# apachepinot/pinot

Measured on AMD Instinct MI355X. Metric: rows scanned/sec, 1B-row segment filter+groupby (3 predicates, SUM/MAX GROUP BY g1), higher is better.
Workload: dtype int64; 1 GPU; 1 segment(s) x 1000000000 rows, one per GPU; SELECT g1, SUM(m), MAX(m) FROM gpuBench WHERE c_inv1 IN (0,1,2,3) AND c_inv2 IN (0,1) AND r_int BETWEEN 250000 AND 749999 GROUP BY g1 ORDER BY g1 LIMIT 1000; query=cfg3, parallelism=segment-per-gpu x1, merge=none (1 segment), entries_scanned_in_filter=249990290

## Files before the change

pinot_amd/csrc/pg_kernels_spec.hip:

```cpp
#define PG_WAVES_PER_BLOCK 12
#define PG_KERNEL template <int PG_NOT_INSTANTIATED> static
#include "pg_kernels.hip"

#define SPEC_LOADERS 4
#ifndef SPEC_TILES
#define SPEC_TILES 2
#endif
#ifndef SPEC_SETS
#define SPEC_SETS 2
#endif
#define SPEC_CONSUMERS 8
#define SPEC_OFF_LIN 0u
#define SPEC_OFF_RNG 256u
#define SPEC_OFF_VAL (256u + 2048u)
#define SPEC_OFF_G0 (256u + 2048u + 8192u)
extern "C" const int pg_spec_waves_per_block = PG_WAVES_PER_BLOCK;
extern "C" int pg_spec_stage_bytes(int bits0, int bits1) { return SPEC_TILES * (((int)SPEC_OFF_G0 + bits0 * 256 + 16 + (bits1 > 0 ? bits1 * 256 + 16 : 0) + 15) & ~15); }

DEVFN void spec_barrier() {
  __builtin_amdgcn_fence(__ATOMIC_RELEASE, "workgroup", "local");
  __builtin_amdgcn_s_barrier();
  __builtin_amdgcn_fence(__ATOMIC_ACQUIRE, "workgroup", "local");
}

template <typename T> DEVFN const GAS T* spec_sgpr_ptr(const void* ptr) {
  const uint64_t v = (uint64_t)ptr;
  const uint32_t lo = (uint32_t)__builtin_amdgcn_readfirstlane((int)(uint32_t)v), hi = (uint32_t)__builtin_amdgcn_readfirstlane((int)(uint32_t)(v >> 32));
  return (const GAS T*)(((uint64_t)hi << 32) | (uint64_t)lo);
}

template <int W> struct SpecCol;
template <> struct SpecCol<0> {};
template <> struct SpecCol<32> { u32x4 r[2]; };
template <> struct SpecCol<24> { u32x4 lo; u32x2 hi; };
template <> struct SpecCol<16> { u32x4 lo; };
template <> struct SpecCol<8> { u32x2 hi; };
constexpr uint32_t spec_img_tile_bytes(int W) { return (uint32_t)(PG_WAVE_DOCS / 8) * (uint32_t)W; }
template <int W> DEVFN void spec_load(SpecCol<W>& c, const uint8_t* base, int wt, int w, int lane) {
  if constexpr (W == 32) {
#pragma unroll
    for (int s = 0; s < 2; s++) {
      const uint8_t* row = base + (size_t)wt * (PG_WAVE_DOCS * 4) + (size_t)(4 * s + w) * 1024u;
      c.r[s] = ldnt((const GAS u32x4*)(spec_sgpr_ptr<uint8_t>(row) + (uint32_t)lane * 16u));
    }
  } else if constexpr (W != 0) {
    const uint8_t* tile = base + (size_t)wt * spec_img_tile_bytes(W);
    if constexpr (W >= 16) c.lo = ldnt((const GAS u32x4*)(spec_sgpr_ptr<uint8_t>(tile + (size_t)w * 1024u) + (uint32_t)lane * 16u));
    if constexpr (W != 16) c.hi = ldnt((const GAS u32x2*)(spec_sgpr_ptr<uint8_t>(tile + (W == 24 ? 4096u : 0u) + (size_t)w * 512u) + (uint32_t)lane * 8u));
  }
}
template <int W> DEVFN void spec_unpack(const SpecCol<W>& c, uint32_t (&a)[4], uint32_t (&b)[4]) {
  if constexpr (W == 32) {
    a[0] = bswap32(c.r[0].x); a[1] = bswap32(c.r[0].y); a[2] = bswap32(c.r[0].z); a[3] = bswap32(c.r[0].w);
    b[0] = bswap32(c.r[1].x); b[1] = bswap32(c.r[1].y); b[2] = bswap32(c.r[1].z); b[3] = bswap32(c.r[1].w);
  } else if constexpr (W == 24) {
    a[0] = __builtin_amdgcn_perm(c.hi.x, c.lo.x, 0x0c040100u); a[1] = __builtin_amdgcn_perm(c.hi.x, c.lo.x, 0x0c050302u);
    a[2] = __builtin_amdgcn_perm(c.hi.x, c.lo.y, 0x0c060100u); a[3] = __builtin_amdgcn_perm(c.hi.x, c.lo.y, 0x0c070302u);
    b[0] = __builtin_amdgcn_perm(c.hi.y, c.lo.z, 0x0c040100u); b[1] = __builtin_amdgcn_perm(c.hi.y, c.lo.z, 0x0c050302u);
    b[2] = __builtin_amdgcn_perm(c.hi.y, c.lo.w, 0x0c060100u); b[3] = __builtin_amdgcn_perm(c.hi.y, c.lo.w, 0x0c070302u);
  } else if constexpr (W == 16) {
    a[0] = c.lo.x & 0xFFFFu; a[1] = c.lo.x >> 16; a[2] = c.lo.y & 0xFFFFu; a[3] = c.lo.y >> 16;
    b[0] = c.lo.z & 0xFFFFu; b[1] = c.lo.z >> 16; b[2] = c.lo.w & 0xFFFFu; b[3] = c.lo.w >> 16;
  } else if constexpr (W == 8) {
#pragma unroll
    for (int e = 0; e < 4; e++) { a[e] = (c.hi.x >> (8 * e)) & 0xFFu; b[e] = (c.hi.y >> (8 * e)) & 0xFFu; }
  }
}
template <int SW, int VW> struct SpecTile {
  SpecCol<SW> scan;
  SpecCol<VW> val;
  u32x4 grp;
};
template <int SW, int VW> struct SpecStage { SpecTile<SW, VW> tile[SPEC_TILES]; uint32_t post[8]; uint32_t tail; };
template <int NG> struct SpecQuad {
  uint32_t lin, rng;
  u32x4 val;
  uint32_t win[NG][2];
};

template <int W> struct SpecWidth { static constexpr int value = W; };
template <int NG, bool HAS_INDEX, bool HAS_SCAN, bool HAS_TAIL = false, bool NARROW = false>
__device__ __forceinline__ void spec_body(const PgQueryPlan& p) {
  extern __shared__ __attribute__((aligned(16))) uint64_t smem[];
  __shared__ uint32_t s_stat[PG_MAX_STATS];
  const int t = threadIdx.x;
  const int lane = t & 63;
  const int wave = uniform(t >> 6);
  int64_t* lds_table = reinterpret_cast<int64_t*>(smem);
  if (t < PG_MAX_STATS) s_stat[t] = 0;
  const uint32_t real_slots = (uint32_t)p.n_groups * (uint32_t)p.replicas;
  const uint32_t table_slots = real_slots + 64u;
  for (int o = 0; o < p.n_ops; o++) {
    const int64_t ident = pg_acc_identity(p.ops[o].fn, p.ops[o].is_float);
    for (uint32_t i = t; i < table_slots; i += PG_BLOCK) lds_table[(size_t)o * table_slots + i] = ident;
  }
  const uint32_t bits0 = (uint32_t)p.gcols[0].bits, bits1 = NG > 1 ? (uint32_t)p.gcols[NG - 1].bits : 0u;
  const uint32_t off_g1 = SPEC_OFF_G0 + bits0 * 256u + 16u;
  const uint32_t tile_bytes = (off_g1 + (NG > 1 ? bits1 * 256u + 16u : 0u) + 15u) & ~15u;
  const uint32_t stage_bytes = tile_bytes * SPEC_TILES;
  uint8_t* stage0 = reinterpret_cast<uint8_t*>(smem) + (((size_t)p.n_ops * table_slots * 8u + 15u) & ~(size_t)15u);
  const CAS PgScanLeaf& L = cptr(p.scans)[HAS_SCAN ? p.fast_scan : 0];
  const int grid = (int)gridDim.x;
  const int n_mine = (int)blockIdx.x < p.n_wtiles ? (p.n_wtiles - (int)blockIdx.x + grid - 1) / grid : 0;
  const int n_stages = (n_mine + SPEC_TILES - 1) / SPEC_TILES;
  __syncthreads();

  if (wave < SPEC_LOADERS) {
    const int w = wave;
    const uint8_t* const xdata = p.srcs[p.pipe_src].data;
    const uint8_t* const simg = NARROW ? p.spec_simg : nullptr;
    const uint8_t* const vimg = NARROW ? p.spec_vimg : nullptr;
    const uint32_t img_slo = NARROW ? p.spec_slo : 0u, img_sspan = NARROW ? p.spec_sspan : 0u, img_vmin = NARROW ? (uint32_t)p.spec_vmin : 0u;
    const bool img_sempty = NARROW && p.spec_sempty != 0;
    const int ggi = (w >> 1) < NG ? (w >> 1) : 0;
    const uint8_t* const gdata = p.gcols[ggi].data;
    const uint32_t gbits = (uint32_t)p.gcols[ggi].bits;
    const uint32_t goff = (uint32_t)(w & 1) * 1024u + (uint32_t)lane * 16u;
    const uint32_t geff = (w >> 1) < NG && goff < gbits * 256u ? goff : 0u;
    const uint8_t* dense_ptr[8];
    int dense_group[8];
#pragma unroll
    for (int j = 0; j < 8; j++) { dense_ptr[j] = HAS_INDEX ? p.dense_ptr[j] : nullptr; dense_group[j] = HAS_INDEX ? p.dense_group[j] : 0; }
    const int dense_groups = p.dense_groups, dense_excl = p.dense_excl;
    const uint8_t* const pipe_tail = HAS_TAIL ? p.pipe_tail : nullptr;
    const int num_docs = p.num_docs;
    const bool scan_pushed = p.fast_scan_pushed != 0;
   auto loaders = [&](auto scan_w, auto val_w) __attribute__((always_inline)) {
    constexpr int SW = HAS_SCAN ? decltype(scan_w)::value : 0, VW = decltype(val_w)::value;
    const RangeI32 r32 = !HAS_SCAN ? RangeI32{0, 0u, false} : (SW == 32 ? make_range_i32(L.lo, L.hi) : RangeI32{(int32_t)img_slo, img_sspan, img_sempty});
    const uint8_t* sdata = !HAS_SCAN ? nullptr : (SW == 32 ? L.data : simg);
    const uint8_t* vdata = VW == 32 ? xdata : vimg;
    const uint32_t vmin = VW == 32 ? 0u : img_vmin;
    uint32_t ld_cand = 0;
    auto issue = [&](int sidx, SpecStage<SW, VW>& st) __attribute__((always_inline)) {
#pragma unroll
      for (int tt = 0; tt < SPEC_TILES; tt++) {
        const int i = sidx * SPEC_TILES + tt;
        const int wt = (int)blockIdx.x + (i < n_mine ? i : n_mine - 1) * grid;
        SpecTile<SW, VW>& tl = st.tile[tt];
        __builtin_amdgcn_sched_barrier(0);
        spec_load<SW>(tl.scan, sdata, wt, w, lane);
        spec_load<VW>(tl.val, vdata, wt, w, lane);
        __builtin_amdgcn_sched_barrier(0);
        {
          const uint8_t* base = gdata + (size_t)wt * (size_t)(PG_WAVE_DOCS / 8) * (size_t)gbits;
          tl.grp = ldnt((const GAS u32x4*)(spec_sgpr_ptr<uint8_t>(base) + geff));
        }
        __builtin_amdgcn_sched_barrier(0);
      }
      if (HAS_INDEX) {
        const int i = sidx * SPEC_TILES + (w % SPEC_TILES);
        const int wt = (int)blockIdx.x + (i < n_mine ? i : n_mine - 1) * grid;
#pragma unroll
        for (int j = 0; j < 8; j++) st.post[j] = *(const GAS uint32_t*)(spec_sgpr_ptr<uint8_t>(dense_ptr[j] + (size_t)wt * 256u) + (uint32_t)lane * 4u);
        __builtin_amdgcn_sched_barrier(0);
      }
      if (HAS_TAIL) {
        const int i = sidx * SPEC_TILES + (w % SPEC_TILES);
        const int wt = (int)blockIdx.x + (i < n_mine ? i : n_mine - 1) * grid;
        st.tail = *(const GAS uint32_t*)(spec_sgpr_ptr<uint8_t>(pipe_tail + (size_t)wt * 256u) + (uint32_t)lane * 4u);
        __builtin_amdgcn_sched_barrier(0);
      }
    };
    auto publish = [&](uint8_t* stage, const SpecStage<SW, VW>& st) __attribute__((always_inline)) {
#ifdef PG_SPEC_NO_PUBLISH
      {
        uint32_t acc = 0;
#pragma unroll
        for (int tt = 0; tt < SPEC_TILES; tt++) {
          uint32_t a[4] = {0u, 0u, 0u, 0u}, b[4] = {0u, 0u, 0u, 0u};
          spec_unpack<SW>(st.tile[tt].scan, a, b); acc += a[0] ^ b[3];
          spec_unpack<VW>(st.tile[tt].val, a, b); acc += a[0] ^ b[3];
          acc += st.tile[tt].grp.x;
        }
        if (acc == 0x12345678u) *reinterpret_cast<uint32_t*>(stage) = acc;
        return;
      }
#endif
#pragma unroll
      for (int tt = 0; tt < SPEC_TILES; tt++) {
        uint8_t* buf = stage + (uint32_t)tt * tile_bytes;
        const SpecTile<SW, VW>& tl = st.tile[tt];
        if (HAS_SCAN) {
          uint32_t q[2][4];
          spec_unpack<SW>(tl.scan, q[0], q[1]);
#pragma unroll
          for (int s = 0; s < 2; s++) {
            uint32_t m = (uint32_t)in_range_i32(r32, (int32_t)q[s][0]) | ((uint32_t)in_range_i32(r32, (int32_t)q[s][1]) << 1) |
                         ((uint32_t)in_range_i32(r32, (int32_t)q[s][2]) << 2) | ((uint32_t)in_range_i32(r32, (int32_t)q[s][3]) << 3);
            m = r32.empty ? 0u : m;
            *reinterpret_cast<uint32_t*>(buf + SPEC_OFF_RNG + (uint32_t)(4 * s + w) * 256u + (uint32_t)lane * 4u) = m;
          }
        }
        {
          uint32_t q[2][4];
          spec_unpack<VW>(tl.val, q[0], q[1]);
#pragma unroll
          for (int s = 0; s < 2; s++) {
            u32x4 v;
            v.x = q[s][0] + vmin; v.y = q[s][1] + vmin; v.z = q[s][2] + vmin; v.w = q[s][3] + vmin;
            *reinterpret_cast<u32x4*>(buf + SPEC_OFF_VAL + (uint32_t)(4 * s + w) * 1024u + (uint32_t)lane * 16u) = v;
          }
        }
        *reinterpret_cast<u32x4*>(buf + (ggi == 0 ? SPEC_OFF_G0 : off_g1) + geff) = tl.grp;
      }
    };
    auto publish_lin = [&](uint8_t* stage, const SpecStage<SW, VW>& st, int sidx) __attribute__((always_inline)) {
      if (w >= SPEC_TILES) return;
      const int i = sidx * SPEC_TILES + w;
      const int wt = (int)blockIdx.x + i * grid;
      const int64_t rem = i < n_mine ? (int64_t)num_docs - (int64_t)wt * PG_WAVE_DOCS : 0;
      const int32_t n_valid = rem >= PG_WAVE_DOCS ? PG_WAVE_DOCS : (rem > 0 ? (int32_t)rem : 0);
      uint32_t lin = valid_lin_mask(n_valid, lane);
      if (HAS_INDEX) {
        uint32_t grp[4] = {0u, 0u, 0u, 0u};
#pragma unroll
        for (int j = 0; j < 8; j++) {
          const int gj = dense_group[j];
#pragma unroll
          for (int k = 0; k < 4; k++) grp[k] |= gj == k ? st.post[j] : 0u;
        }
#pragma unroll
        for (int k = 0; k < 4; k++)
          if (k < dense_groups) lin &= ((dense_excl >> k) & 1) ? ~grp[k] : grp[k];
      }
      *reinterpret_cast<uint32_t*>(stage + (uint32_t)w * tile_bytes + SPEC_OFF_LIN + (uint32_t)lane * 4u) = HAS_TAIL ? lin & st.tail : lin;
      ld_cand += (uint32_t)__popc(lin);
    };
    constexpr int SETS = HAS_SCAN ? SPEC_SETS : 2 * SPEC_SETS;
    SpecStage<SW, VW> st[SETS];
    auto buf_of = [&](int sg) __attribute__((always_inline)) { return stage0 + (uint32_t)(sg & 1) * stage_bytes; };
    if (n_stages > 0) {
#pragma unroll
      for (int k = 0; k < SETS; k++) issue(k, st[k]);
    }
    int s = 0;
    for (; s + SETS - 1 < n_stages; s += SETS) {
#pragma unroll
      for (int k = 0; k < SETS; k++) {
        publish(buf_of(s + k), st[k]);
        publish_lin(buf_of(s + k), st[k], s + k);
        issue(s + k + SETS, st[k]);
        spec_barrier();
      }
    }
#pragma unroll
    for (int k = 0; k < SETS - 1; k++)
      if (s + k < n_stages) {
        publish(buf_of(s + k), st[k]);
        publish_lin(buf_of(s + k), st[k], s + k);
        spec_barrier();
      }
    const uint32_t csum = wave_sum_u32(ld_cand);
    if (HAS_SCAN && !scan_pushed && lane == 0 && csum) atomicAdd(&s_stat[L.stat_slot], csum);
   };
    if constexpr (!NARROW) {
      loaders(SpecWidth<32>{}, SpecWidth<32>{});
    } else {
      const int sb = uniform(p.spec_sbits), vb = uniform(p.spec_vbits);
      auto with_scan = [&](auto scan_w) __attribute__((always_inline)) {
        switch (vb) {
          case 8: loaders(scan_w, SpecWidth<8>{}); break;
          case 16: loaders(scan_w, SpecWidth<16>{}); break;
          case 24: loaders(scan_w, SpecWidth<24>{}); break;
          default: loaders(scan_w, SpecWidth<32>{}); break;
        }
      };
      switch (sb) {
        case 8: with_scan(SpecWidth<8>{}); break;
        case 16: with_scan(SpecWidth<16>{}); break;
        case 24: with_scan(SpecWidth<24>{}); break;
        default: with_scan(SpecWidth<32>{}); break;
      }
    }
  } else {
    const int c = wave - SPEC_LOADERS;
    const uint32_t R = (uint32_t)p.replicas;
    const uint32_t rep = (uint32_t)t & (R - 1u);
    const uint32_t stride = table_slots;
    const uint32_t trash_slot = real_slots + (uint32_t)lane;
    const uint32_t q = (uint32_t)c * 64u + (uint32_t)lane;
    const uint32_t nib = ((uint32_t)lane & 7u) * 4u;
    uint32_t my_matched = 0;
    const int n_ops = uniform(p.n_ops);
    uint64_t ops_code = 0;
    for (int o = 0; o < n_ops; o++) {
      const PgAccOp op = p.ops[uniform(o)];
      ops_code |= (uint64_t)(op.src < 0 ? 0u : (op.fn == PG_ACC_SUM ? 1u : (op.fn == PG_ACC_MIN ? 2u : 3u))) << (2 * o);
    }
    ops_code = ((uint64_t)(uint32_t)uniform((int)(uint32_t)(ops_code >> 32)) << 32) | (uint64_t)(uint32_t)uniform((int)(uint32_t)ops_code);
    const int has_out_words = uniform(p.out_words != nullptr ? 1 : 0);
    auto fetch = [&](const uint8_t* buf, SpecQuad<NG>& d) __attribute__((always_inline)) {
      d.lin = *reinterpret_cast<const uint32_t*>(buf + SPEC_OFF_LIN + (q >> 3) * 4u);
      d.rng = HAS_SCAN ? *reinterpret_cast<const uint32_t*>(buf + SPEC_OFF_RNG + q * 4u) : 0xFu;
      d.val = *reinterpret_cast<const u32x4*>(buf + SPEC_OFF_VAL + q * 16u);
#pragma unroll
      for (int gi = 0; gi < NG; gi++) {
        const uint32_t di = __umul24(4u * q, (uint32_t)p.gcols[gi].bits) >> 5;
        const uint32_t* win = reinterpret_cast<const uint32_t*>(buf + (gi == 0 ? SPEC_OFF_G0 : off_g1)) + di;
        d.win[gi][0] = win[0]; d.win[gi][1] = win[1];
      }
    };
    auto aggregate = [&](const SpecQuad<NG> (&d)[SPEC_TILES], int sidx) __attribute__((always_inline)) {
      constexpr int ND = 4 * SPEC_TILES;
      uint32_t slot[ND];
      int32_t v[ND];
#pragma unroll
      for (int tt = 0; tt < SPEC_TILES; tt++) {
        const int i = sidx * SPEC_TILES + tt;
        const uint32_t cand = (d[tt].lin >> nib) & 0xFu;
        const uint32_t m = d[tt].rng & cand;
        my_matched += (uint32_t)__popc(m);
        if (has_out_words && i < n_mine) {
          const int wt = (int)blockIdx.x + i * grid;
          const uint32_t word = or_reduce8(m << nib);
          if ((lane & 7) == 0) reinterpret_cast<uint32_t*>(p.out_words)[(int64_t)wt * 64 + (int64_t)(q >> 3)] = word;
        }
#ifndef PG_SPEC_NO_TABLE
#pragma unroll
        for (int e = 0; e < 4; e++) slot[4 * tt + e] = rep;
#pragma unroll
        for (int gi = 0; gi < NG; gi++) {
          const PgGroupCol& gc = p.gcols[gi];
          const uint32_t bits = (uint32_t)gc.bits, mask = (1u << gc.bits) - 1u;
          const uint32_t mult = (uint32_t)gc.mult * R;
          uint32_t dv[4];
          decode_packed_quad<true>(d[tt].win[gi], q, bits, mask, dv);
#pragma unroll
          for (int e = 0; e < 4; e++) slot[4 * tt + e] += __umul24(dv[e], mult);
        }
#pragma unroll
        for (int e = 0; e < 4; e++) slot[4 * tt + e] = ((m >> e) & 1u) ? slot[4 * tt + e] : trash_slot;
        v[4 * tt + 0] = (int32_t)d[tt].val.x; v[4 * tt + 1] = (int32_t)d[tt].val.y; v[4 * tt + 2] = (int32_t)d[tt].val.z; v[4 * tt + 3] = (int32_t)d[tt].val.w;
#endif
      }
#ifdef PG_SPEC_NO_TABLE
      return;
#endif
      for (int o = 0; o < n_ops; o++) {
        const uint32_t code = (uint32_t)(ops_code >> (2 * o)) & 3u;
        int64_t* base = lds_table + (size_t)o * stride;
        if (code == 0u) {
#pragma unroll
          for (int e = 0; e < ND; e++) atomicAdd(reinterpret_cast<unsigned long long*>(base + slot[e]), 1ULL);
        } else if (code == 1u) {
#pragma unroll
          for (int e = 0; e < ND; e++) atomicAdd(reinterpret_cast<unsigned long long*>(base + slot[e]), (unsigned long long)(int64_t)v[e]);
        } else if (code == 2u) {
#pragma unroll
          for (int e = 0; e < ND; e++) atomicMin(reinterpret_cast<long long*>(base + slot[e]), (long long)v[e]);
        } else {
#pragma unroll
          for (int e = 0; e < ND; e++) atomicMax(reinterpret_cast<long long*>(base + slot[e]), (long long)v[e]);
        }
      }
    };
    auto fetch_stage = [&](int sidx, SpecQuad<NG> (&d)[SPEC_TILES]) __attribute__((always_inline)) {
      const uint8_t* stage = stage0 + (uint32_t)(sidx & 1) * stage_bytes;
#pragma unroll
      for (int tt = 0; tt < SPEC_TILES; tt++) fetch(stage + (uint32_t)tt * tile_bytes, d[tt]);
    };
    auto aggregate_stage = [&](int sidx, const SpecQuad<NG> (&d)[SPEC_TILES]) __attribute__((always_inline)) {
#ifdef PG_SPEC_NO_CONSUME
      return;
#endif
#ifdef PG_SPEC_FETCH_ONLY
      {
        uint32_t acc = 0;
#pragma unroll
        for (int tt = 0; tt < SPEC_TILES; tt++) { acc += d[tt].lin ^ d[tt].rng ^ d[tt].val.x ^ d[tt].val.w; for (int gi = 0; gi < NG; gi++) acc += d[tt].win[gi][0] ^ d[tt].win[gi][1]; }
        if (acc == 0x12345678u) my_matched++;
        return;
      }
#endif
      aggregate(d, sidx);
    };
    SpecQuad<NG> da[SPEC_TILES], db[SPEC_TILES];
    if (n_stages > 0) {
      spec_barrier();
#ifndef PG_SPEC_NO_CONSUME
      fetch_stage(0, da);
#endif
    }
    for (int s = 0; s < n_stages; s += 2) {
      if (s + 1 < n_stages) {
        spec_barrier();
#ifndef PG_SPEC_NO_CONSUME
        fetch_stage(s + 1, db);
#endif
      }
      aggregate_stage(s, da);
      if (s + 1 < n_stages) {
        if (s + 2 < n_stages) {
          spec_barrier();
#ifndef PG_SPEC_NO_CONSUME
          fetch_stage(s + 2, da);
#endif
        }
        aggregate_stage(s + 1, db);
      }
    }
    const uint32_t wsum = wave_sum_u32(my_matched);
    if (lane == 0 && wsum) atomicAdd(&s_stat[0], wsum);
  }
  __syncthreads();
  if (t < PG_MAX_STATS && s_stat[t]) atomicAdd(&p.stats[t], (unsigned long long)s_stat[t]);
  {
    const int R = p.replicas, groups = p.n_groups;
    int64_t* out = p.partials + (int64_t)blockIdx.x * ((int64_t)p.n_ops * groups);
    for (int o = 0; o < p.n_ops; o++) {
      const int fn = p.ops[uniform(o)].fn;
      for (int gq = t; gq < groups; gq += PG_BLOCK) {
        const int64_t* src = lds_table + (size_t)o * table_slots + (size_t)gq * R;
        int64_t acc = src[0];
        if (fn == PG_ACC_COUNT || fn == PG_ACC_SUM) { for (int r = 1; r < R; r++) acc += src[r]; }
        else if (fn == PG_ACC_MIN) { for (int r = 1; r < R; r++) acc = src[r] < acc ? src[r] : acc; }
        else { for (int r = 1; r < R; r++) acc = src[r] > acc ? src[r] : acc; }
        out[(size_t)o * groups + gq] = acc;
      }
    }
  }
}
#define PG_SPEC_KERNEL(NAME, IDX, SCAN) \
  extern "C" __global__ void __launch_bounds__(PG_BLOCK) NAME(const PgQueryPlan p) { \
    if (p.n_group_cols == 1) spec_body<1, IDX, SCAN>(p); \
    else spec_body<2, IDX, SCAN>(p); \
  }
PG_SPEC_KERNEL(pg_spec_none, false, false)
PG_SPEC_KERNEL(pg_spec_scan, false, true)
PG_SPEC_KERNEL(pg_spec_index, true, false)
#undef PG_SPEC_KERNEL
extern "C" __global__ void __launch_bounds__(PG_BLOCK) pg_fast_i32range_s(const PgQueryPlan p) {
  if (p.n_group_cols == 1) spec_body<1, true, true, false, true>(p);
  else spec_body<2, true, true, false, true>(p);
}
extern "C" __global__ void __launch_bounds__(PG_BLOCK) pg_fast_i32range_st(const PgQueryPlan p) {
  if (p.n_group_cols == 1) spec_body<1, true, true, true, true>(p);
  else spec_body<2, true, true, true, true>(p);
}
```

pinot_amd/csrc/pg_segment.cpp:

```cpp
#include <hip/hip_runtime.h>

#include <algorithm>
#include <cmath>

#include "pg_internal.hpp"

extern "C" __global__ void __launch_bounds__(256) pg_column_magnitude_kernel(const uint8_t* __restrict__ data, int64_t n, int val_type,
                                                                             unsigned long long* __restrict__ out) {
  unsigned long long mx = 0, bad = 0;
  for (int64_t i = (int64_t)blockIdx.x * blockDim.x + threadIdx.x; i < n; i += (int64_t)gridDim.x * blockDim.x) {
    unsigned long long a;
    if (val_type == PG_V_I64) {
      const unsigned long long v = __builtin_bswap64(reinterpret_cast<const unsigned long long*>(data)[i]);
      a = (long long)v < 0 ? 0ULL - v : v;
    } else {
      double d;
      if (val_type == PG_V_F32) d = (double)__uint_as_float(__builtin_bswap32(reinterpret_cast<const uint32_t*>(data)[i]));
      else d = __longlong_as_double((long long)__builtin_bswap64(reinterpret_cast<const unsigned long long*>(data)[i]));
      a = (unsigned long long)__double_as_longlong(d) & 0x7FFFFFFFFFFFFFFFULL;
      if (a >= 0x7FF0000000000000ULL) { bad = 1; a = 0; }
    }
    mx = a > mx ? a : mx;
  }
  for (int off = 32; off > 0; off >>= 1) {
    const unsigned long long o = __shfl_xor(mx, off, 64);
    mx = o > mx ? o : mx;
    bad |= __shfl_xor(bad, off, 64);
  }
  if ((threadIdx.x & 63) == 0) {
    if (mx) atomicMax(&out[0], mx);
    if (bad) atomicOr(&out[1], 1ULL);
  }
}

extern "C" __global__ void __launch_bounds__(256) pg_column_int_range_kernel(const uint8_t* __restrict__ data, int64_t n, int val_type,
                                                                             long long* __restrict__ out) {
  long long mn = INT64_MAX, mx = INT64_MIN;
  for (int64_t i = (int64_t)blockIdx.x * blockDim.x + threadIdx.x; i < n; i += (int64_t)gridDim.x * blockDim.x) {
    const long long v = val_type == PG_V_I64 ? (long long)__builtin_bswap64(reinterpret_cast<const unsigned long long*>(data)[i])
                                             : (long long)(int32_t)__builtin_bswap32(reinterpret_cast<const uint32_t*>(data)[i]);
    mn = v < mn ? v : mn;
    mx = v > mx ? v : mx;
  }
  for (int off = 32; off > 0; off >>= 1) {
    const long long a = __shfl_xor(mn, off, 64), b = __shfl_xor(mx, off, 64);
    mn = a < mn ? a : mn;
    mx = b > mx ? b : mx;
  }
  if ((threadIdx.x & 63) == 0 && mn <= mx) {
    atomicMin(&out[0], mn);
    atomicMax(&out[1], mx);
  }
}

extern "C" __global__ void __launch_bounds__(256) pg_column_narrow_image_kernel(const uint8_t* __restrict__ data, uint8_t* __restrict__ img,
                                                                                int64_t n_wtiles, int32_t vmin, int bits) {
  const int64_t n = n_wtiles * 256;
  const int64_t tile_bytes = (int64_t)(PG_WAVE_DOCS / 8) * bits;
  for (int64_t i = (int64_t)blockIdx.x * blockDim.x + threadIdx.x; i < n; i += (int64_t)gridDim.x * blockDim.x) {
    const int64_t wt = i >> 8;
    const int b = (int)(i >> 6) & 3, l = (int)i & 63;
    const uint4 qa = *reinterpret_cast<const uint4*>(data + wt * (PG_WAVE_DOCS * 4) + (int64_t)b * 1024 + l * 16);
    const uint4 qb = *reinterpret_cast<const uint4*>(data + wt * (PG_WAVE_DOCS * 4) + (int64_t)(4 + b) * 1024 + l * 16);
    const uint32_t raw[8] = {qa.x, qa.y, qa.z, qa.w, qb.x, qb.y, qb.z, qb.w};
    uint32_t s[8];
    for (int e = 0; e < 8; e++) s[e] = (__builtin_bswap32(raw[e]) - (uint32_t)vmin) & (bits == 24 ? 0xFFFFFFu : (bits == 16 ? 0xFFFFu : 0xFFu));
    uint8_t* tile = img + wt * tile_bytes;
    if (bits >= 16) {
      uint4 lo;
      lo.x = (s[0] & 0xFFFFu) | (s[1] << 16); lo.y = (s[2] & 0xFFFFu) | (s[3] << 16);
      lo.z = (s[4] & 0xFFFFu) | (s[5] << 16); lo.w = (s[6] & 0xFFFFu) | (s[7] << 16);
      *reinterpret_cast<uint4*>(tile + (int64_t)b * 1024 + l * 16) = lo;
    }
    if (bits != 16) {
      const int sh = bits == 24 ? 16 : 0;
      uint2 hi;
      hi.x = ((s[0] >> sh) & 0xFFu) | (((s[1] >> sh) & 0xFFu) << 8) | (((s[2] >> sh) & 0xFFu) << 16) | (((s[3] >> sh) & 0xFFu) << 24);
      hi.y = ((s[4] >> sh) & 0xFFu) | (((s[5] >> sh) & 0xFFu) << 8) | (((s[6] >> sh) & 0xFFu) << 16) | (((s[7] >> sh) & 0xFFu) << 24);
      *reinterpret_cast<uint2*>(tile + (bits == 24 ? 4096 : 0) + (int64_t)b * 512 + l * 8) = hi;
    }
  }
}

extern "C" __global__ void __launch_bounds__(256) pg_column_max_dict_id_kernel(const uint8_t* __restrict__ data, int64_t n, int bits,
                                                                                unsigned int* __restrict__ out) {
  unsigned int mx = 0;
  const uint64_t mask = (1ULL << bits) - 1ULL;
  for (int64_t i = (int64_t)blockIdx.x * blockDim.x + threadIdx.x; i < n; i += (int64_t)gridDim.x * blockDim.x) {
    const uint64_t bit = (uint64_t)i * (uint64_t)bits;
    const uint8_t* p = data + (bit >> 3);
    uint64_t w = 0;
    for (int k = 0; k < 8; k++) w = (w << 8) | p[k];
    const unsigned int v = (unsigned int)((w >> (64 - bits - (int)(bit & 7))) & mask);
    mx = v > mx ? v : mx;
  }
  for (int off = 32; off > 0; off >>= 1) {
    const unsigned int o = __shfl_xor(mx, off, 64);
    mx = o > mx ? o : mx;
  }
  if ((threadIdx.x & 63) == 0 && mx) atomicMax(out, mx);
}

namespace pg {

static int32_t fx_exp_of(double max_abs) {
  if (!(max_abs > 0)) return 0;
  int e = 0;
  (void)std::frexp(max_abs, &e);
  return (int32_t)(16 * (int)std::floor(((double)e + 15.0) / 16.0));
}

static inline uint32_t be32(const uint8_t* p) {
  return ((uint32_t)p[0] << 24) | ((uint32_t)p[1] << 16) | ((uint32_t)p[2] << 8) | (uint32_t)p[3];
}
static inline uint64_t be64(const uint8_t* p) { return ((uint64_t)be32(p) << 32) | be32(p + 4); }
static inline uint16_t le16(const uint8_t* p) { return (uint16_t)(p[0] | (p[1] << 8)); }
static inline uint32_t le32(const uint8_t* p) {
  return (uint32_t)p[0] | ((uint32_t)p[1] << 8) | ((uint32_t)p[2] << 16) | ((uint32_t)p[3] << 24);
}

Column* Segment::find(const char* n) {
  if (!n) return nullptr;
  auto it = columns.find(n);
  return it == columns.end() ? nullptr : it->second.get();
}

static size_t padded_docs(const Segment& seg) { return (size_t)seg.n_tiles * PG_TILE_DOCS; }

static void check_dict_ids(const Column& c, int64_t n) {
  if (n <= 0 || c.cardinality <= 0 || !(c.bits >= 31 || ((int64_t)1 << c.bits) > (int64_t)c.cardinality)) return;
  DeviceBuffer out(4, true);
  const int grid = (int)std::max<int64_t>(1, std::min<int64_t>(2048, (n + 255) / 256));
  hipLaunchKernelGGL(pg_column_max_dict_id_kernel, dim3(grid), dim3(256), 0, 0, c.fwd_dev.as<uint8_t>(), n, c.bits, out.as<unsigned int>());
  PG_HIP(hipGetLastError());
  unsigned int mx = 0;
  PG_HIP(hipMemcpy(&mx, out.ptr, 4, hipMemcpyDeviceToHost));
  if ((int64_t)mx >= (int64_t)c.cardinality)
    fail(PG_ERR_INVALID_ARGUMENT, "forward index of %s holds dictId %u, the dictionary has %d values", c.name.c_str(), mx, c.cardinality);
}

static void upload_fixed_bit(Segment& seg, Column& c, const uint8_t* src, uint64_t len) {
  uint64_t need = ((uint64_t)seg.total_docs * (uint64_t)c.bits + 7) / 8;
  if (len < need) fail(PG_ERR_INVALID_ARGUMENT, "forward index of %s is %llu bytes, need %llu", c.name.c_str(),
                       (unsigned long long)len, (unsigned long long)need);
  size_t alloc = (padded_docs(seg) * (size_t)c.bits + 7) / 8 + 64;
  c.fwd_dev.alloc(alloc, true);
  c.fwd_dev.upload(src, need);
  c.col_kind = PG_COL_FIXED_BIT;
  c.fwd_bytes_logical = need;
  check_dict_ids(c, (int64_t)seg.total_docs);
}

static void parse_inverted_index(Segment& seg, Column& c, const uint8_t* inv, uint64_t len) {
  const int32_t card = c.cardinality;
  const uint64_t off_end = ((uint64_t)card + 1) * 4;
  if (len < off_end) fail(PG_ERR_INVALID_ARGUMENT, "inverted index of %s too short", c.name.c_str());
  const uint64_t first = be32(inv);
  const uint8_t* bitmap_buffer = inv + off_end;
  c.posting_begin.assign((size_t)card + 1, 0);
  std::vector<uint8_t> staging;
  staging.reserve(len);
  const uint32_t max_key = (uint32_t)((padded_docs(seg) + PG_CHUNK_DOCS - 1) / PG_CHUNK_DOCS);
  c.posting_card.assign((size_t)card, 0);
  for (int32_t d = 0; d < card; d++) {
    c.posting_begin[d] = (uint32_t)c.descs_host.size();
    uint64_t off = be32(inv + (uint64_t)d * 4), end = be32(inv + (uint64_t)(d + 1) * 4);
    if (end < off || off < first || (end - first) > len - off_end)
      fail(PG_ERR_INVALID_ARGUMENT, "inverted index of %s: bad offsets for dictId %d", c.name.c_str(), d);
    const uint8_t* blob = bitmap_buffer + (off - first);
    uint64_t blen = end - off;
    if (blen < 8) fail(PG_ERR_INVALID_ARGUMENT, "roaring blob too short (%s dictId %d)", c.name.c_str(), d);
    uint32_t cookie = le32(blob);
    uint64_t pos = 4;
    uint32_t size;
    const uint8_t* run_flags = nullptr;
    bool has_run = false;
    if ((cookie & 0xFFFF) == 12347) {
      size = (cookie >> 16) + 1;
      run_flags = blob + pos;
      pos += (size + 7) / 8;
      has_run = true;
    } else if (cookie == 12346) {
      size = le32(blob + pos);
      pos += 4;
    } else {
      fail(PG_ERR_INVALID_ARGUMENT, "roaring: bad cookie %u (%s dictId %d)", cookie, c.name.c_str(), d);
    }
    if (pos + 4ULL * size > blen) fail(PG_ERR_INVALID_ARGUMENT, "roaring: truncated header");
    const uint8_t* desc = blob + pos;
    pos += 4ULL * size;
    if (!has_run || size >= 4) pos += 4ULL * size;
    for (uint32_t i = 0; i < size; i++) {
      PgContainer pc{};
      pc.key = le16(desc + 4 * i);
      uint32_t cardm1 = le16(desc + 4 * i + 2);
      bool is_run = has_run && ((run_flags[i >> 3] >> (i & 7)) & 1);
      uint64_t payload;
      if (is_run) {
        if (pos + 2 > blen) fail(PG_ERR_INVALID_ARGUMENT, "roaring: truncated run container");
        pc.n = le16(blob + pos);
        pos += 2;
        pc.type = 2;
        payload = 4ULL * pc.n;
      } else if (cardm1 + 1 > 4096) {
        pc.type = 1;
        pc.n = cardm1 + 1;
        payload = 8192;
      } else {
        pc.type = 0;
        pc.n = cardm1 + 1;
        payload = 2ULL * pc.n;
      }
      if (pos + payload > blen) fail(PG_ERR_INVALID_ARGUMENT, "roaring: truncated container");
      if (pc.type == 2) for (uint32_t r = 0; r < pc.n; r++) c.posting_card[(size_t)d] += (int64_t)le16(blob + pos + 4 * r + 2) + 1;
      else c.posting_card[(size_t)d] += pc.n;
      if (pc.key >= max_key) fail(PG_ERR_INVALID_ARGUMENT, "roaring: container key %u beyond the segment", pc.key);
      size_t aligned = (staging.size() + 15) & ~(size_t)15;
      staging.resize(aligned + payload);
      memcpy(staging.data() + aligned, blob + pos, payload);
      pc.offset = aligned;
      pos += payload;
      c.descs_host.push_back(pc);
    }
  }
  c.posting_begin[card] = (uint32_t)c.descs_host.size();
  staging.resize(((staging.size() + 15) & ~(size_t)15) + 16);
  c.containers_dev.alloc(staging.size());
  c.containers_dev.upload(staging.data(), staging.size());
  c.descs_dev = upload_vector(c.descs_host);
  c.has_inverted = true;
}

static std::shared_ptr<Column> bitmap_column(Segment& seg, const std::string& name, const void* roaring, uint64_t size) {
  if (!roaring || size < 8) fail(PG_ERR_INVALID_ARGUMENT, "%s: not a serialized RoaringBitmap", name.c_str());
  if (size > 0xFFFFFFF0ULL) fail(PG_ERR_UNSUPPORTED, "%s: bitmap larger than 4 GB", name.c_str());
  auto col = std::make_shared<Column>();
  col->name = name;
  col->cardinality = 1;
  std::vector<uint8_t> inv(8 + size);
  const uint32_t offs[2] = {8, (uint32_t)(8 + size)};
  for (int i = 0; i < 2; i++) for (int b = 0; b < 4; b++) inv[(size_t)i * 4 + b] = (uint8_t)(offs[i] >> (24 - 8 * b));
  memcpy(inv.data() + 8, roaring, size);
  parse_inverted_index(seg, *col, inv.data(), inv.size());
  return col;
}

void segment_set_null_vector(Segment& seg, const char* column, const void* roaring, uint64_t size) {
  if (!column || !seg.find(column)) fail(PG_ERR_NOT_FOUND, "column not found: %s", column ? column : "(null)");
  auto col = bitmap_column(seg, std::string("nullvalue_vector of ") + column, roaring, size);
  std::lock_guard<std::mutex> g(seg.mu);
  seg.null_vectors[column] = std::move(col);
  seg.plan_cache.clear();
}

void segment_set_range_index(Segment& seg, const char* column, const void* bytes, uint64_t size) {
  Column* c = column ? seg.find(column) : nullptr;
  if (!c) fail(PG_ERR_NOT_FOUND, "column not found: %s", column ? column : "(null)");
  const uint8_t* p = static_cast<const uint8_t*>(bytes);
  if (!p || size < 22) fail(PG_ERR_INVALID_ARGUMENT, "range index of %s too short", column);
  const int32_t version = (int32_t)be32(p);
  if (version != 2) fail(PG_ERR_UNSUPPORTED, "range index of %s: version %d (only the exact bit-sliced index, version 2, is on the GPU path)", column, version);
  const int64_t min = (int64_t)be64(p + 4);
  const uint8_t* r = p + 12;
  if (le16(r) != 0xF00D || r[2] != 2) fail(PG_ERR_INVALID_ARGUMENT, "range index of %s: bad RangeBitmap cookie / base", column);
  const int slices = r[3];
  const uint32_t max_key = le16(r + 4), max_rid = le32(r + 6);
  const int bytes_per_mask = (slices + 7) >> 3;
  if (slices < 1 || slices > 64) fail(PG_ERR_INVALID_ARGUMENT, "range index of %s: %d slices", column, slices);
  if ((int64_t)max_rid < (int64_t)seg.total_docs) fail(PG_ERR_INVALID_ARGUMENT, "range index of %s covers %u rows, the segment has %d", column, max_rid, seg.total_docs);
  const uint32_t n_chunks = (uint32_t)((padded_docs(seg) + PG_CHUNK_DOCS - 1) / PG_CHUNK_DOCS);
  if (max_key > n_chunks) fail(PG_ERR_INVALID_ARGUMENT, "range index of %s: %u chunks beyond the segment", column, max_key);
  uint64_t pos = 22 + (uint64_t)max_key * (uint64_t)bytes_per_mask;
  if (pos > size) fail(PG_ERR_INVALID_ARGUMENT, "range index of %s: truncated masks", column);
  std::vector<PgContainer> descs((size_t)n_chunks * (size_t)slices);
  for (auto& d : descs) { d.offset = 0; d.n = 0; d.key = 0; d.type = 3; }
  std::vector<uint8_t> staging;
  staging.reserve(size);
  for (uint32_t key = 0; key < max_key; key++) {
    uint64_t mask = 0;
    for (int b = 0; b < bytes_per_mask; b++) mask |= (uint64_t)p[22 + (uint64_t)key * bytes_per_mask + b] << (8 * b);
    for (int s = 0; s < slices; s++) {
      if (!((mask >> s) & 1)) continue;
      if (pos + 1 > size) fail(PG_ERR_INVALID_ARGUMENT, "range index of %s: truncated container", column);
      const int type = p[pos++];
      PgContainer pc{};
      pc.key = (uint16_t)key;
      uint64_t payload;
      if (type == 0) { pc.type = 1; pc.n = 0; payload = 8192; }
      else if (type == 1 || type == 2) {
        if (pos + 2 > size) fail(PG_ERR_INVALID_ARGUMENT, "range index of %s: truncated container", column);
        pc.n = le16(p + pos);
        pos += 2;
        pc.type = type == 1 ? 2 : 0;
        payload = type == 1 ? 4ULL * pc.n : 2ULL * pc.n;
      } else {
        fail(PG_ERR_INVALID_ARGUMENT, "range index of %s: container type %d", column, type);
      }
      if (pos + payload > size) fail(PG_ERR_INVALID_ARGUMENT, "range index of %s: truncated container", column);
      const size_t aligned = (staging.size() + 15) & ~(size_t)15;
      staging.resize(aligned + payload);
      memcpy(staging.data() + aligned, p + pos, payload);
      pc.offset = aligned;
      pos += payload;
      descs[(size_t)key * (size_t)slices + (size_t)s] = pc;
    }
  }
  staging.resize(((staging.size() + 15) & ~(size_t)15) + 16);
  DeviceBuffer cont(staging.size());
  cont.upload(staging.data(), staging.size());
  DeviceBuffer dd = upload_vector(descs);
  std::lock_guard<std::mutex> g(seg.mu);
  seg.device_bytes += cont.size + dd.size;
  c->ri_containers_dev = std::move(cont);
  c->ri_descs_dev = std::move(dd);
  c->ri_slices = slices;
  c->ri_chunks = (int32_t)n_chunks;
  c->ri_min = min;
  c->ri_bytes = size;
  c->has_range_index = true;
  seg.plan_cache.clear();
}

void segment_set_queryable_doc_ids(Segment& seg, const void* roaring, uint64_t size) {
  std::shared_ptr<Column> col;
  if (size) col = bitmap_column(seg, "queryableDocIds", roaring, size);
  std::lock_guard<std::mutex> g(seg.mu);
  seg.queryable_doc_ids = std::move(col);
  seg.plan_cache.clear();
}

template <typename F>
static void walk_var_byte_chunks(const Segment& seg, const uint8_t* fwd, uint64_t fwd_len, const char* name, bool pass_through_only, F each) {
  if (fwd_len < 28) fail(PG_ERR_INVALID_ARGUMENT, "raw forward index of %s too short", name);
  const int32_t version = (int32_t)be32(fwd), num_chunks = (int32_t)be32(fwd + 4), per_chunk = (int32_t)be32(fwd + 8);
  if (version != 2 && version != 3) fail(PG_ERR_UNSUPPORTED, "column %s: var-byte chunk writer version %d", name, version);
  const int32_t longest = (int32_t)be32(fwd + 12), compression = (int32_t)be32(fwd + 20), header_start = (int32_t)be32(fwd + 24);
  if (compression != 0 && pass_through_only)
    fail(PG_ERR_UNSUPPORTED, "column %s: compressed var-byte chunks (type %d) are outside the GPU path", name, compression);
  const int off_size = version == 2 ? 4 : 8;
  if (per_chunk <= 0 || num_chunks < 0 || longest < 0 || (int64_t)num_chunks * per_chunk < seg.total_docs || header_start < 28 ||
      (uint64_t)header_start + (uint64_t)num_chunks * (uint64_t)off_size > fwd_len)
    fail(PG_ERR_INVALID_ARGUMENT, "raw forward index of %s: %d chunks of %d docs for %d docs", name, num_chunks, per_chunk, seg.total_docs);
  const uint64_t max_chunk = (uint64_t)per_chunk * (4ULL + (uint64_t)longest);
  for (int32_t ch = 0; ch < num_chunks && (int64_t)ch * per_chunk < seg.total_docs; ch++) {
    auto chunk_pos = [&](int32_t i) -> uint64_t {
      if (i == num_chunks) return fwd_len;
      const uint8_t* o = fwd + header_start + (uint64_t)i * (uint64_t)off_size;
      return off_size == 4 ? (uint64_t)be32(o) : be64(o);
    };
    const uint64_t start = chunk_pos(ch), end = chunk_pos(ch + 1);
    if (start > end || end > fwd_len) fail(PG_ERR_INVALID_ARGUMENT, "raw forward index of %s: bad chunk offsets", name);
    std::vector<uint8_t> plain;
    const uint8_t* cb = fwd + start;
    uint64_t clen = end - start;
    if (compression != 0) {
      plain = host_decompress_chunk(compression, cb, clen, max_chunk, name);
      cb = plain.data();
      clen = plain.size();
    }
    if (clen < (uint64_t)per_chunk * 4) fail(PG_ERR_INVALID_ARGUMENT, "raw forward index of %s: chunk %d is %llu bytes", name, ch, (unsigned long long)clen);
    const int32_t rows = (int32_t)std::min<int64_t>(per_chunk, (int64_t)seg.total_docs - (int64_t)ch * per_chunk);
    for (int32_t r = 0; r < rows; r++) {
      const uint64_t vs = be32(cb + (size_t)r * 4);
      uint64_t ve = clen;
      if (r + 1 < per_chunk) { const uint64_t nx = be32(cb + (size_t)(r + 1) * 4); if (nx != 0) ve = nx; }
      if (vs < (uint64_t)per_chunk * 4 || ve < vs || ve > clen) fail(PG_ERR_INVALID_ARGUMENT, "raw forward index of %s: bad value offsets in chunk %d", name, ch);
      each((int64_t)ch * per_chunk + r, cb + vs, ve - vs);
    }
  }
}

void segment_add_column(Segment& seg, const pg_column_desc& d) {
  if (!d.name) fail(PG_ERR_INVALID_ARGUMENT, "column name is null");
  if (seg.columns.count(d.name)) fail(PG_ERR_INVALID_ARGUMENT, "column %s already added", d.name);
  auto col = std::make_unique<Column>();
  Column& c = *col;
  c.name = d.name;
  c.data_type = d.data_type;
  c.fwd_encoding = d.fwd_encoding;
  c.has_dictionary = d.has_dictionary != 0;
  c.cardinality = d.cardinality;
  c.bits = d.bits_per_value;
// ... 569 lines not shown
```

Baseline: 841.6 billion rows/s.

## Split narrow-image loaders by column and widen hi-byte loads to 16B

For narrow (8/16/24-bit) column images, the four loader waves are now split by column: two waves load the scan column and two load the value column, each covering one whole tile of a stage. Previously each loader loaded a slice of both columns. The image builder interleaves the high-byte plane so each lane can fetch it with 16-byte loads instead of 8-byte ones. The goal is fewer, wider global loads per wave and less unpack work per column. The cost is uneven work between the two roles, since only one role does the index/tail loads, and more registers held per stage.

Result: faster. 870.4 billion rows/s (median of 6 runs) (+3.4%).

```diff
diff --git a/pinot_amd/csrc/pg_kernels_spec.hip b/pinot_amd/csrc/pg_kernels_spec.hip
--- a/pinot_amd/csrc/pg_kernels_spec.hip
+++ b/pinot_amd/csrc/pg_kernels_spec.hip
@@ -8,6 +8,9 @@
 #endif
 #ifndef SPEC_SETS
 #define SPEC_SETS 2
+#endif
+#ifndef SPEC_INDEX_ROLE
+#define SPEC_INDEX_ROLE 0
 #endif
 #define SPEC_CONSUMERS 8
 #define SPEC_OFF_LIN 0u
@@ -32,9 +35,6 @@
 template <int W> struct SpecCol;
 template <> struct SpecCol<0> {};
 template <> struct SpecCol<32> { u32x4 r[2]; };
-template <> struct SpecCol<24> { u32x4 lo; u32x2 hi; };
-template <> struct SpecCol<16> { u32x4 lo; };
-template <> struct SpecCol<8> { u32x2 hi; };
 constexpr uint32_t spec_img_tile_bytes(int W) { return (uint32_t)(PG_WAVE_DOCS / 8) * (uint32_t)W; }
 template <int W> DEVFN void spec_load(SpecCol<W>& c, const uint8_t* base, int wt, int w, int lane) {
   if constexpr (W == 32) {
@@ -43,29 +43,53 @@
       const uint8_t* row = base + (size_t)wt * (PG_WAVE_DOCS * 4) + (size_t)(4 * s + w) * 1024u;
       c.r[s] = ldnt((const GAS u32x4*)(spec_sgpr_ptr<uint8_t>(row) + (uint32_t)lane * 16u));
     }
-  } else if constexpr (W != 0) {
-    const uint8_t* tile = base + (size_t)wt * spec_img_tile_bytes(W);
-    if constexpr (W >= 16) c.lo = ldnt((const GAS u32x4*)(spec_sgpr_ptr<uint8_t>(tile + (size_t)w * 1024u) + (uint32_t)lane * 16u));
-    if constexpr (W != 16) c.hi = ldnt((const GAS u32x2*)(spec_sgpr_ptr<uint8_t>(tile + (W == 24 ? 4096u : 0u) + (size_t)w * 512u) + (uint32_t)lane * 8u));
   }
 }
 template <int W> DEVFN void spec_unpack(const SpecCol<W>& c, uint32_t (&a)[4], uint32_t (&b)[4]) {
   if constexpr (W == 32) {
     a[0] = bswap32(c.r[0].x); a[1] = bswap32(c.r[0].y); a[2] = bswap32(c.r[0].z); a[3] = bswap32(c.r[0].w);
     b[0] = bswap32(c.r[1].x); b[1] = bswap32(c.r[1].y); b[2] = bswap32(c.r[1].z); b[3] = bswap32(c.r[1].w);
+  }
+}
+template <int W> struct SpecColT;
+template <> struct SpecColT<32> { u32x4 r[8]; };
+template <> struct SpecColT<24> { u32x4 lo[4]; u32x4 hi[2]; };
+template <> struct SpecColT<16> { u32x4 lo[4]; };
+template <> struct SpecColT<8> { u32x4 hi[2]; };
+template <int W> DEVFN void spec_load_tile(SpecColT<W>& c, const uint8_t* base, int wt, int lane) {
+  const GAS uint8_t* tile = spec_sgpr_ptr<uint8_t>(base + (size_t)wt * spec_img_tile_bytes(W));
+  if constexpr (W == 32) {
+#pragma unroll
+    for (int r = 0; r < 8; r++) c.r[r] = ldnt((const GAS u32x4*)(tile + (uint32_t)r * 1024u + (uint32_t)lane * 16u));
+  } else {
+    if constexpr (W >= 16) {
+#pragma unroll
+      for (int b = 0; b < 4; b++) c.lo[b] = ldnt((const GAS u32x4*)(tile + (uint32_t)b * 1024u + (uint32_t)lane * 16u));
+    }
+    if constexpr (W != 16) {
+#pragma unroll
+      for (int h = 0; h < 2; h++) c.hi[h] = ldnt((const GAS u32x4*)(tile + (W == 24 ? 4096u : 0u) + (uint32_t)h * 1024u + (uint32_t)lane * 16u));
+    }
+  }
+}
+template <int W, int R> DEVFN void spec_unpack_tile(const SpecColT<W>& c, uint32_t (&q)[4]) {
+  constexpr int B = R & 3, S = R >> 2;
+  if constexpr (W == 32) {
+    q[0] = bswap32(c.r[R].x); q[1] = bswap32(c.r[R].y); q[2] = bswap32(c.r[R].z); q[3] = bswap32(c.r[R].w);
   } else if constexpr (W == 24) {
-    a[0] = __builtin_amdgcn_perm(c.hi.x, c.lo.x, 0x0c040100u); a[1] = __builtin_amdgcn_perm(c.hi.x, c.lo.x, 0x0c050302u);
-    a[2] = __builtin_amdgcn_perm(c.hi.x, c.lo.y, 0x0c060100u); a[3] = __builtin_amdgcn_perm(c.hi.x, c.lo.y, 0x0c070302u);
-    b[0] = __builtin_amdgcn_perm(c.hi.y, c.lo.z, 0x0c040100u); b[1] = __builtin_amdgcn_perm(c.hi.y, c.lo.z, 0x0c050302u);
-    b[2] = __builtin_amdgcn_perm(c.hi.y, c.lo.w, 0x0c060100u); b[3] = __builtin_amdgcn_perm(c.hi.y, c.lo.w, 0x0c070302u);
+    const uint32_t l0 = c.lo[B][2 * S], l1 = c.lo[B][2 * S + 1], h = c.hi[B >> 1][2 * (B & 1) + S];
+    q[0] = __builtin_amdgcn_perm(h, l0, 0x0c040100u); q[1] = __builtin_amdgcn_perm(h, l0, 0x0c050302u);
+    q[2] = __builtin_amdgcn_perm(h, l1, 0x0c060100u); q[3] = __builtin_amdgcn_perm(h, l1, 0x0c070302u);
   } else if constexpr (W == 16) {
-    a[0] = c.lo.x & 0xFFFFu; a[1] = c.lo.x >> 16; a[2] = c.lo.y & 0xFFFFu; a[3] = c.lo.y >> 16;
-    b[0] = c.lo.z & 0xFFFFu; b[1] = c.lo.z >> 16; b[2] = c.lo.w & 0xFFFFu; b[3] = c.lo.w >> 16;
-  } else if constexpr (W == 8) {
-#pragma unroll
-    for (int e = 0; e < 4; e++) { a[e] = (c.hi.x >> (8 * e)) & 0xFFu; b[e] = (c.hi.y >> (8 * e)) & 0xFFu; }
-  }
-}
+    const uint32_t l0 = c.lo[B][2 * S], l1 = c.lo[B][2 * S + 1];
+    q[0] = l0 & 0xFFFFu; q[1] = l0 >> 16; q[2] = l1 & 0xFFFFu; q[3] = l1 >> 16;
+  } else {
+    const uint32_t h = c.hi[B >> 1][2 * (B & 1) + S];
+#pragma unroll
+    for (int e = 0; e < 4; e++) q[e] = (h >> (8 * e)) & 0xFFu;
+  }
+}
+template <int W> struct SpecColStage { SpecColT<W> col; u32x4 grp[SPEC_TILES]; uint32_t post[8]; uint32_t tail; };
 template <int SW, int VW> struct SpecTile {
   SpecCol<SW> scan;
   SpecCol<VW> val;
@@ -254,23 +278,147 @@
     const uint32_t csum = wave_sum_u32(ld_cand);
     if (HAS_SCAN && !scan_pushed && lane == 0 && csum) atomicAdd(&s_stat[L.stat_slot], csum);
    };
+   auto col_loaders = [&](auto role_c, auto width_c) __attribute__((always_inline)) {
+    static_assert(SPEC_TILES == 2 && SPEC_LOADERS == 4 && HAS_SCAN, "column loaders: 2 columns x 2 tiles of a stage over 4 loaders");
+    constexpr int ROLE = decltype(role_c)::value, W = decltype(width_c)::value;
+    const RangeI32 r32 = W == 32 ? make_range_i32(L.lo, L.hi) : RangeI32{(int32_t)img_slo, img_sspan, img_sempty};
+    const uint8_t* cdata = ROLE == 0 ? (W == 32 ? L.data : simg) : (W == 32 ? xdata : vimg);
+    const uint32_t vmin = W == 32 ? 0u : img_vmin;
+    const int tw = w & 1;
+    uint32_t ld_cand = 0;
+    auto tile_of = [&](int sidx, int tt) __attribute__((always_inline)) {
+      const int i = sidx * SPEC_TILES + tt;
+      return (int)blockIdx.x + (i < n_mine ? i : n_mine - 1) * grid;
+    };
+    auto issue = [&](int sidx, SpecColStage<W>& st) __attribute__((always_inline)) {
+      __builtin_amdgcn_sched_barrier(0);
+      spec_load_tile<W>(st.col, cdata, tile_of(sidx, tw), lane);
+      __builtin_amdgcn_sched_barrier(0);
+#pragma unroll
+      for (int tt = 0; tt < SPEC_TILES; tt++) {
+        const uint8_t* base = gdata + (size_t)tile_of(sidx, tt) * (size_t)(PG_WAVE_DOCS / 8) * (size_t)gbits;
+        st.grp[tt] = ldnt((const GAS u32x4*)(spec_sgpr_ptr<uint8_t>(base) + geff));
+      }
+      __builtin_amdgcn_sched_barrier(0);
+      if constexpr (ROLE == SPEC_INDEX_ROLE) {
+        const int wt = tile_of(sidx, tw);
+        if (HAS_INDEX) {
+#pragma unroll
+          for (int j = 0; j < 8; j++) st.post[j] = ldnt((const GAS uint32_t*)(spec_sgpr_ptr<uint8_t>(dense_ptr[j] + (size_t)wt * 256u) + (uint32_t)lane * 4u));
+          __builtin_amdgcn_sched_barrier(0);
+        }
+        if (HAS_TAIL) {
+          st.tail = ldnt((const GAS uint32_t*)(spec_sgpr_ptr<uint8_t>(pipe_tail + (size_t)wt * 256u) + (uint32_t)lane * 4u));
+          __builtin_amdgcn_sched_barrier(0);
+        }
+      }
+    };
+    auto publish = [&](uint8_t* stage, const SpecColStage<W>& st) __attribute__((always_inline)) {
+#ifdef PG_SPEC_NO_PUBLISH
+      {
+        uint32_t acc = 0, a[4], b[4];
+        spec_unpack_tile<W, 0>(st.col, a); spec_unpack_tile<W, 3>(st.col, b); acc += a[0] ^ b[3];
+        spec_unpack_tile<W, 5>(st.col, a); spec_unpack_tile<W, 6>(st.col, b); acc += a[0] ^ b[3];
+#pragma unroll
+        for (int tt = 0; tt < SPEC_TILES; tt++) acc += st.grp[tt].x;
+        if (acc == 0x12345678u) *reinterpret_cast<uint32_t*>(stage) = acc;
+        return;
+      }
+#endif
+      uint8_t* buf = stage + (uint32_t)tw * tile_bytes;
+      auto row = [&](auto row_c) __attribute__((always_inline)) {
+        constexpr int R = decltype(row_c)::value;
+        uint32_t q[4];
+        spec_unpack_tile<W, R>(st.col, q);
+        if constexpr (ROLE == 0) {
+          uint32_t m = (uint32_t)in_range_i32(r32, (int32_t)q[0]) | ((uint32_t)in_range_i32(r32, (int32_t)q[1]) << 1) |
+                       ((uint32_t)in_range_i32(r32, (int32_t)q[2]) << 2) | ((uint32_t)in_range_i32(r32, (int32_t)q[3]) << 3);
+          m = r32.empty ? 0u : m;
+          *reinterpret_cast<uint32_t*>(buf + SPEC_OFF_RNG + (uint32_t)R * 256u + (uint32_t)lane * 4u) = m;
+        } else {
+          u32x4 v;
+          v.x = q[0] + vmin; v.y = q[1] + vmin; v.z = q[2] + vmin; v.w = q[3] + vmin;
+          *reinterpret_cast<u32x4*>(buf + SPEC_OFF_VAL + (uint32_t)R * 1024u + (uint32_t)lane * 16u) = v;
+        }
+      };
+      row(SpecWidth<0>{}); row(SpecWidth<1>{}); row(SpecWidth<2>{}); row(SpecWidth<3>{});
+      row(SpecWidth<4>{}); row(SpecWidth<5>{}); row(SpecWidth<6>{}); row(SpecWidth<7>{});
+#pragma unroll
+      for (int tt = 0; tt < SPEC_TILES; tt++)
+        *reinterpret_cast<u32x4*>(stage + (uint32_t)tt * tile_bytes + (ggi == 0 ? SPEC_OFF_G0 : off_g1) + geff) = st.grp[tt];
+    };
+    auto publish_lin = [&](uint8_t* stage, const SpecColStage<W>& st, int sidx) __attribute__((always_inline)) {
+      if constexpr (ROLE == SPEC_INDEX_ROLE) {
+        const int i = sidx * SPEC_TILES + tw;
+        const int wt = (int)blockIdx.x + i * grid;
+        const int64_t rem = i < n_mine ? (int64_t)num_docs - (int64_t)wt * PG_WAVE_DOCS : 0;
+        const int32_t n_valid = rem >= PG_WAVE_DOCS ? PG_WAVE_DOCS : (rem > 0 ? (int32_t)rem : 0);
+        uint32_t lin = valid_lin_mask(n_valid, lane);
+        if (HAS_INDEX) {
+          uint32_t grp[4] = {0u, 0u, 0u, 0u};
+#pragma unroll
+          for (int j = 0; j < 8; j++) {
+            const int gj = dense_group[j];
+#pragma unroll
+            for (int k = 0; k < 4; k++) grp[k] |= gj == k ? st.post[j] : 0u;
+          }
+#pragma unroll
+          for (int k = 0; k < 4; k++)
+            if (k < dense_groups) lin &= ((dense_excl >> k) & 1) ? ~grp[k] : grp[k];
+        }
+        *reinterpret_cast<uint32_t*>(stage + (uint32_t)tw * tile_bytes + SPEC_OFF_LIN + (uint32_t)lane * 4u) = HAS_TAIL ? lin & st.tail : lin;
+        ld_cand += (uint32_t)__popc(lin);
+      }
+    };
+    SpecColStage<W> st[SPEC_SETS];
+    auto buf_of = [&](int sg) __attribute__((always_inline)) { return stage0 + (uint32_t)(sg & 1) * stage_bytes; };
+    if (n_stages > 0) {
+#pragma unroll
+      for (int k = 0; k < SPEC_SETS; k++) issue(k, st[k]);
+    }
+    int s = 0;
+    for (; s + SPEC_SETS - 1 < n_stages; s += SPEC_SETS) {
+#pragma unroll
+      for (int k = 0; k < SPEC_SETS; k++) {
+        publish(buf_of(s + k), st[k]);
+        publish_lin(buf_of(s + k), st[k], s + k);
+        issue(s + k + SPEC_SETS, st[k]);
+        spec_barrier();
+      }
+    }
+#pragma unroll
+    for (int k = 0; k < SPEC_SETS - 1; k++)
+      if (s + k < n_stages) {
+        publish(buf_of(s + k), st[k]);
+        publish_lin(buf_of(s + k), st[k], s + k);
+        spec_barrier();
+      }
+    if constexpr (ROLE == SPEC_INDEX_ROLE) {
+      const uint32_t csum = wave_sum_u32(ld_cand);
+      if (!scan_pushed && lane == 0 && csum) atomicAdd(&s_stat[L.stat_slot], csum);
+    }
+   };
     if constexpr (!NARROW) {
       loaders(SpecWidth<32>{}, SpecWidth<32>{});
     } else {
       const int sb = uniform(p.spec_sbits), vb = uniform(p.spec_vbits);
-      auto with_scan = [&](auto scan_w) __attribute__((always_inline)) {
+      const bool img_s = sb == 8 || sb == 16 || sb == 24, img_v = vb == 8 || vb == 16 || vb == 24;
+      if (!img_s && !img_v) {
+        loaders(SpecWidth<32>{}, SpecWidth<32>{});
+      } else if ((w >> 1) == 0) {
+        switch (sb) {
+          case 8: col_loaders(SpecWidth<0>{}, SpecWidth<8>{}); break;
+          case 16: col_loaders(SpecWidth<0>{}, SpecWidth<16>{}); break;
+          case 24: col_loaders(SpecWidth<0>{}, SpecWidth<24>{}); break;
+          default: col_loaders(SpecWidth<0>{}, SpecWidth<32>{}); break;
+        }
+      } else {
         switch (vb) {
-          case 8: loaders(scan_w, SpecWidth<8>{}); break;
-          case 16: loaders(scan_w, SpecWidth<16>{}); break;
-          case 24: loaders(scan_w, SpecWidth<24>{}); break;
-          default: loaders(scan_w, SpecWidth<32>{}); break;
-        }
-      };
-      switch (sb) {
-        case 8: with_scan(SpecWidth<8>{}); break;
-        case 16: with_scan(SpecWidth<16>{}); break;
-        case 24: with_scan(SpecWidth<24>{}); break;
-        default: with_scan(SpecWidth<32>{}); break;
+          case 8: col_loaders(SpecWidth<1>{}, SpecWidth<8>{}); break;
+          case 16: col_loaders(SpecWidth<1>{}, SpecWidth<16>{}); break;
+          case 24: col_loaders(SpecWidth<1>{}, SpecWidth<24>{}); break;
+          default: col_loaders(SpecWidth<1>{}, SpecWidth<32>{}); break;
+        }
       }
     }
   } else {
diff --git a/pinot_amd/csrc/pg_segment.cpp b/pinot_amd/csrc/pg_segment.cpp
--- a/pinot_amd/csrc/pg_segment.cpp
+++ b/pinot_amd/csrc/pg_segment.cpp
@@ -77,7 +77,7 @@
       uint2 hi;
       hi.x = ((s[0] >> sh) & 0xFFu) | (((s[1] >> sh) & 0xFFu) << 8) | (((s[2] >> sh) & 0xFFu) << 16) | (((s[3] >> sh) & 0xFFu) << 24);
       hi.y = ((s[4] >> sh) & 0xFFu) | (((s[5] >> sh) & 0xFFu) << 8) | (((s[6] >> sh) & 0xFFu) << 16) | (((s[7] >> sh) & 0xFFu) << 24);
-      *reinterpret_cast<uint2*>(tile + (bits == 24 ? 4096 : 0) + (int64_t)b * 512 + l * 8) = hi;
+      *reinterpret_cast<uint2*>(tile + (bits == 24 ? 4096 : 0) + (int64_t)(b >> 1) * 1024 + l * 16 + (b & 1) * 8) = hi;
     }
   }
 }
```
